# spaceandtimefdn/blitzar

Hardware: NVIDIA H100
Metric: MSM throughput (scalar*point terms/sec), ristretto255, n=2^20 per GPU (higher is better)
Workload: dtype u32 limbs (integer modular arithmetic)

## Files before the change

### blitzar_b200/csrc/msm.cuh

```cuda
#pragma once
#include <algorithm>
#include <vector>

#include "batch_affine.cuh"
#include "curve.cuh"
#include "engine_api.cuh"
#include "lanefield.cuh"

namespace b200 {

struct ColumnDesc {
  const unsigned char* base;
  u64 row_stride;
  u32 bit_offset;
  u32 bit_width;
  u32 n;
  u32 is_signed;
  u32 first_window;
  u32 num_windows;
  u32 table_n;
  u32 gen_base;
};
B200_HD u32 bucket_windows(const ColumnDesc& col) { return col.table_n ? (col.num_windows ? 1u : 0u) : col.num_windows; }

// ... 40 lines not shown
  }
  negative = false;
  if (col.is_signed) {
    u32 top = width - 1;
    bool neg = false;
#pragma unroll
    for (int k = 0; k < 8; ++k)
      if ((top >> 5) == (u32)k)
        neg = (v[k] >> (top & 31u)) & 1u;
    if (neg) {
      u64 c = 1;
#pragma unroll
      for (int k = 0; k < 8; ++k) {
        int lo = 32 * k;
        u32 m = 0;
        if ((int)width >= lo + 32)
          m = 0xffffffffu;
        else if ((int)width > lo)
          m = (1u << (width - lo)) - 1u;
        c += (u64)((~v[k]) & m);
        v[k] = (u32)c & m;
        c = (m == 0xffffffffu) ? (c >> 32) : 0;
      }
      negative = true;
    }
  }
}

constexpr u32 kAllWindows = 0xffffffffu;
template <class Fn>
B200_HD void for_each_digit(const u32 v[8], bool negative, const ColumnDesc& col, u32 c,
                            u32 nbuckets, Fn f, u32 only_window = kAllWindows) {
  const u32 half = nbuckets;
  const u32 mask = (1u << c) - 1u;
  u64 buf = 0;
  u32 nb = 0, w = 0, carry = 0;
  const u32 W = only_window == kAllWindows
                    ? col.num_windows
                    : (only_window < col.num_windows ? only_window + 1 : 0u);
  const auto step = [&] {
    u32 d = ((u32)buf & mask) + carry;
    buf >>= c;
    bool dneg = d > half;
    carry = dneg ? 1u : 0u;
    if (dneg)
      d = (1u << c) - d;
    if (d && (only_window == kAllWindows || w == only_window))
      f((col.first_window + (col.table_n ? 0u : w)) * nbuckets + (d - 1u), negative != dneg, w);
    ++w;
  };
#pragma unroll
  for (int k = 0; k < 8; ++k) {
    buf |= (u64)v[k] << nb;
    nb += 32;
    for (; nb >= c && w < W; nb -= c)
      step();
  }
  while (w < W)
    step();
}

B200_HD u32 column_of(const u64* col_start, u32 ncols, u64 tid) {
  u32 lo = 0, hi = ncols;
  while (hi - lo > 1) {
    const u32 mid = (lo + hi) >> 1;
    if (tid >= col_start[mid])
      lo = mid;
    else
      hi = mid;
  }
  return lo;
}
template <class Fn>
B200_HD void for_each_entry(const ColumnDesc* cols, const u64* col_start, u32 ncols, u32 c,
                            u32 nbuckets, u64 tid, Fn f, u32 only_window = kAllWindows) {
  const u32 j = column_of(col_start, ncols, tid);
  const ColumnDesc col = cols[j];
  if (only_window != kAllWindows && only_window >= col.num_windows)
    return;
  const u64 i = tid - col_start[j];
  u32 v[8];
  bool neg;
  load_scalar_bits(v, neg, col, i);
  const u32 ii = (u32)i + col.gen_base, tn = col.table_n;
  for_each_digit(v, neg, col, c, nbuckets, [&](u32 key, bool negate, u32 w) {
    f(key, make_entry(key, ii + w * tn, negate));
  }, only_window);
}

struct CountBody {
  static constexpr int kBlock = 256;
  const ColumnDesc* cols;
  const u64* col_start;
  u32 ncols, c, nbuckets;
  u32* counts;
  B200_HD void operator()(u64 tid) const {
    u32* cnt = counts;
    for_each_entry(cols, col_start, ncols, c, nbuckets, tid,
                   [cnt](u32 key, u64) { B200_ATOMIC_ADD(&cnt[key], 1u); });
  }
};

struct ScatterBody {
  static constexpr int kBlock = 256;
  const ColumnDesc* cols;
  const u64* col_start;
  u32 ncols, c, nbuckets;
  u32* cursor;
  u64* entries;
  u64 total_terms;
  B200_HD void operator()(u64 tid) const {
    u32 only = kAllWindows;
    if (total_terms) {
      only = (u32)(tid / total_terms);
      tid -= (u64)only * total_terms;
    }
    u32* cur = cursor;
    u64* en = entries;
    for_each_entry(cols, col_start, ncols, c, nbuckets, tid,
                   [cur, en](u32 key, u64 e) { en[B200_ATOMIC_ADD(&cur[key], 1u)] = e; }, only);
  }
};

constexpr u32 kScanChunk = 256, kScanChunkFirst = 64;
struct ScanUpBody {
  static constexpr int kBlock = 128;
  const u32* in;
  u64 n;
  u32* partial;
  u32 chunk;
  B200_HD void operator()(u64 t) const {
    u64 b = t * chunk, e = b + chunk < n ? b + chunk : n;
    u32 s = 0;
    for (u64 i = b; i < e; ++i)
      s += in[i];
    partial[t] = s;
  }
};
struct ScanTopBody {
  static constexpr int kBlock = 32;
  u32* data;
  u64 n;
  B200_HD void operator()(u64) const {
    u32 s = 0;
    for (u64 i = 0; i < n; ++i) {
      u32 v = data[i];
      data[i] = s;
      s += v;
    }
  }
};
struct ScanDownBody {
  static constexpr int kBlock = 128;
  u32* data;
  u64 n;
  const u32* partial_scanned;
  u32 chunk;
  B200_HD void operator()(u64 t) const {
    u64 b = t * chunk, e = b + chunk < n ? b + chunk : n;
    u32 s = partial_scanned[t];
    for (u64 i = b; i < e; ++i) {
      u32 v = data[i];
      data[i] = s;
      s += v;
    }
  }
};

inline void exclusive_scan(u32* data, u64 n, stream_t s, u32 chunk = kScanChunkFirst) {
  if (n <= kScanChunk) {
    launch(ScanTopBody{data, n}, 1, s);
    return;
  }
  u64 m = (n + chunk - 1) / chunk;
  u32* partial = (u32*)dev_alloc(m * sizeof(u32), s);
  launch(ScanUpBody{data, n, partial, chunk}, m, s);
  exclusive_scan(partial, m, s, kScanChunk);
  launch(ScanDownBody{data, n, partial, chunk}, m, s);
  dev_free(partial, s);
}

#if defined(__CUDACC__) && !defined(B200_EMULATE)
#define B200_BINNED_SORT 1
constexpr u32 kMicroBins = 16384, kBinCap = 8192, kBinSpan = 4096, kMaxBinShift = 12;
constexpr u64 kBinnedSortMinEntries = 1ull << 20;

template <int kBlock> __device__ u32 block_exclusive_scan(u32 v, u32* warp_sums, u32* total) {
  const u32 lane = threadIdx.x & 31u, warp = threadIdx.x >> 5;
  u32 x = v;
#pragma unroll
  for (int d = 1; d < 32; d <<= 1) {
    const u32 y = __shfl_up_sync(0xffffffffu, x, d);
    if (lane >= (u32)d)
      x += y;
  }
  if (lane == 31)
    warp_sums[warp] = x;
  __syncthreads();
  if (warp == 0) {
    u32 w = lane < kBlock / 32 ? warp_sums[lane] : 0u;
#pragma unroll
    for (int d = 1; d < 32; d <<= 1) {
      const u32 y = __shfl_up_sync(0xffffffffu, w, d);
      if (lane >= (u32)d)
        w += y;
    }
    if (lane < kBlock / 32)
      warp_sums[lane] = w;
  }
  __syncthreads();
  const u32 pre = (warp ? warp_sums[warp - 1] : 0u) + x - v;
  *total = warp_sums[kBlock / 32 - 1];
  __syncthreads();
  return pre;
}

struct MicroCountBody {
  static constexpr int kBlock = 512;
  const ColumnDesc* cols;
  const u64* col_start;
  u32 ncols, c, nbuckets;
  u64 total_terms;
  u32 tile, shift, nmicro;
  u32* micro_counts;
  __device__ void run(u32 b, unsigned char* smem) const {
    u32* h = (u32*)smem;
    for (u32 m = threadIdx.x; m < nmicro; m += kBlock)
      h[m] = 0;
    __syncthreads();
    const u64 lo = (u64)b * tile, hi = lo + tile < total_terms ? lo + tile : total_terms;
    const u32 sh = shift;
    for (u64 t = lo + threadIdx.x; t < hi; t += kBlock)
      for_each_entry(cols, col_start, ncols, c, nbuckets, t,
                     [h, sh](u32 key, u64) { atomicAdd(&h[key >> sh], 1u); });
    __syncthreads();
    for (u32 m = threadIdx.x; m < nmicro; m += kBlock)
      if (h[m])
        atomicAdd(&micro_counts[m], h[m]);
  }
};

struct PlanBinsBody {
  static constexpr int kBlock = 1024;
  const u32* micro_counts;
  u32 nmicro, span_micro;
  u64 nkeys;
  u32* bin_of;
  u32* bin_start;
  u32* bin_micro;
  u32* bin_cursor;
  u32* nbins_out;
  u32* counts;
  u32* d_m;
  __device__ bool starts_bin(const u32* st, u32 m) const {
    constexpr u32 H = kBinCap / 2;
    return m == 0 || m % span_micro == 0 || micro_counts[m] > H || micro_counts[m - 1] > H ||
           st[m] / H != st[m - 1] / H;
  }
  __device__ void run(u32, unsigned char* smem) const {
    __shared__ u32 ws[32];
    u32* st = (u32*)smem;
    const u32 per = (nmicro + kBlock - 1) / kBlock, m0 = min(threadIdx.x * per, nmicro),
              m1 = min(m0 + per, nmicro);
    u32 sum = 0;
    for (u32 m = m0; m < m1; ++m)
      sum += micro_counts[m];
    u32 total;
    u32 run = block_exclusive_scan<kBlock>(sum, ws, &total);
    for (u32 m = m0; m < m1; ++m) {
      st[m] = run;
      run += micro_counts[m];
    }
    __syncthreads();
    u32 nf = 0;
    for (u32 m = m0; m < m1; ++m)
      nf += starts_bin(st, m) ? 1u : 0u;
    u32 nbins;
    u32 id = block_exclusive_scan<kBlock>(nf, ws, &nbins);
    for (u32 m = m0; m < m1; ++m) {
      if (starts_bin(st, m)) {
        bin_start[id] = st[m];
        bin_micro[id] = m;
        bin_cursor[id] = st[m];
        ++id;
      }
      bin_of[m] = id - 1;
    }
    if (threadIdx.x == 0) {
      bin_start[nbins] = total;
      bin_micro[nbins] = nmicro;
      *nbins_out = nbins;
      counts[nkeys] = total;
      d_m[0] = total;
    }
  }
};

struct CoarseScatterBody {
  static constexpr int kBlock = 1024;
  const ColumnDesc* cols;
  const u64* col_start;
  u32 ncols, c, nbuckets;
  u64 total_terms;
  u32 tile, shift, nmicro;
  const u32* bin_of;
  const u32* nbins_ptr;
  u32* bin_cursor;
  u64* tmp;
  __device__ void run(u32 b, unsigned char* smem) const {
    __shared__ u32 ws[32];
    u32* h = (u32*)smem;
    u32* delta = h + nmicro;
    u64* stage = (u64*)(delta + nmicro + (nmicro & 1u));
    const u32 nbins = *nbins_ptr;
    for (u32 k = threadIdx.x; k < nbins; k += kBlock)
      h[k] = 0;
    __syncthreads();
    const u64 lo = (u64)b * tile, hi = lo + tile < total_terms ? lo + tile : total_terms;
    const u32 sh = shift;
    const u32* map = bin_of;
    for (u64 t = lo + threadIdx.x; t < hi; t += kBlock)
      for_each_entry(cols, col_start, ncols, c, nbuckets, t,
                     [h, sh, map](u32 key, u64) { atomicAdd(&h[__ldg(&map[key >> sh])], 1u); });
    __syncthreads();
    const u32 per = (nbins + kBlock - 1) / kBlock, k0 = min(threadIdx.x * per, nbins),
              k1 = min(k0 + per, nbins);
    u32 sum = 0;
    for (u32 k = k0; k < k1; ++k)
      sum += h[k];
    u32 size;
    u32 run = block_exclusive_scan<kBlock>(sum, ws, &size);
    for (u32 k = k0; k < k1; ++k) {
      const u32 n = h[k];
      if (n)
        delta[k] = atomicAdd(&bin_cursor[k], n) - run;
      h[k] = run;
      run += n;
    }
    __syncthreads();
    for (u64 t = lo + threadIdx.x; t < hi; t += kBlock)
      for_each_entry(cols, col_start, ncols, c, nbuckets, t, [h, sh, map, stage](u32 key, u64 e) {
        stage[atomicAdd(&h[__ldg(&map[key >> sh])], 1u)] = e;
      });
    __syncthreads();
    for (u32 i = threadIdx.x; i < size; i += kBlock) {
      const u64 e = stage[i];
      tmp[delta[__ldg(&map[entry_key(e) >> sh])] + i] = e;
    }
  }
};

struct BinSortBody {
  static constexpr int kBlock = 1024;
  static constexpr size_t kSmem = 2 * kBinCap * sizeof(u64) + kBinSpan * sizeof(u32);
  const u64* tmp;
  const u32* bin_start;
  const u32* bin_micro;
  const u32* nbins_ptr;
  u32 shift;
  u64 nkeys;
  u64* entries;
  u32* counts;
  __device__ void run(u32 b, unsigned char* smem) const {
    __shared__ u32 ws[32];
    if (b >= *nbins_ptr)
      return;
    u64* ent = (u64*)smem;
    u32* h = (u32*)(smem + 2 * kBinCap * sizeof(u64));
    const u32 lo = bin_start[b], size = bin_start[b + 1] - lo;
    const u64 klo = (u64)bin_micro[b] << shift, khi_m = (u64)bin_micro[b + 1] << shift;
    const u32 span = (u32)((khi_m < nkeys ? khi_m : nkeys) - klo);
    const bool local = size <= kBinCap;
    for (u32 k = threadIdx.x; k < span; k += kBlock)
      h[k] = 0;
    if (local) {
#pragma unroll 4
      for (u32 i = threadIdx.x; i < size; i += kBlock)
        ent[i] = tmp[(u64)lo + i];
    }
    __syncthreads();
    for (u32 i = threadIdx.x; i < size; i += kBlock) {
      const u64 e = local ? ent[i] : tmp[(u64)lo + i];
      atomicAdd(&h[entry_key(e) - (u32)klo], 1u);
    }
    __syncthreads();
    const u32 per = (span + kBlock - 1) / kBlock, k0 = min(threadIdx.x * per, span),
              k1 = min(k0 + per, span);
    u32 sum = 0;
    for (u32 k = k0; k < k1; ++k)
      sum += h[k];
    u32 total;
    u32 run = block_exclusive_scan<kBlock>(sum, ws, &total);
    for (u32 k = k0; k < k1; ++k) {
      const u32 n = h[k];
      h[k] = run;
      run += n;
      counts[klo + k] = lo + run;
    }
    __syncthreads();
    if (!local) {
      for (u32 i = threadIdx.x; i < size; i += kBlock) {
        const u64 e = tmp[(u64)lo + i];
        entries[(u64)lo + atomicAdd(&h[entry_key(e) - (u32)klo], 1u)] = e;
      }
      return;
    }
    u64* sorted = ent + kBinCap;
    for (u32 i = threadIdx.x; i < size; i += kBlock) {
      const u64 e = ent[i];
      sorted[atomicAdd(&h[entry_key(e) - (u32)klo], 1u)] = e;
    }
    __syncthreads();
    for (u32 i = threadIdx.x; i < size; i += kBlock)
      entries[(u64)lo + i] = sorted[i];
  }
};

inline u32 binned_sort_shift(u64 nkeys) {
  u32 shift = 0;
  while ((nkeys + (1ull << shift) - 1) >> shift > kMicroBins)
    ++shift;
  return shift;
}

inline void binned_sort(stream_t s, const ColumnDesc* d_cols, const u64* d_col_start, u32 ncols,
                        u32 c, u32 nbuckets, u64 total_terms, u64 max_entries, u32 max_windows,
                        u64 nkeys, u64* entries, u32* counts, u32* d_m) {
  const u32 shift = binned_sort_shift(nkeys);
  const u32 nmicro = (u32)((nkeys + (1ull << shift) - 1) >> shift);
  const u32 span_micro = std::max(1u, kBinSpan >> shift);
  u32* ws = (u32*)dev_alloc((5ull * nmicro + 3) * sizeof(u32), s);
  u32 *micro_counts = ws, *bin_of = ws + nmicro, *bin_cursor = ws + 2ull * nmicro,
      *bin_start = ws + 3ull * nmicro, *bin_micro = ws + 4ull * nmicro + 1,
      *nbins = ws + 5ull * nmicro + 2;
  u64* tmp = (u64*)dev_alloc(std::max<u64>(max_entries, 1) * sizeof(u64), s);
  dev_zero(micro_counts, nmicro * sizeof(u32), s);
  const u64 count_tile = 4096;
  launch_blocks(MicroCountBody{d_cols, d_col_start, ncols, c, nbuckets, total_terms,
                               (u32)count_tile, shift, nmicro, micro_counts},
                (total_terms + count_tile - 1) / count_tile, nmicro * sizeof(u32), s);
  launch_blocks(PlanBinsBody{micro_counts, nmicro, span_micro, nkeys, bin_of, bin_start, bin_micro,
                             bin_cursor, nbins, counts, d_m},
                1, nmicro * sizeof(u32), s);
  const size_t scatter_smem = 220 * 1024;
  const size_t bin_bytes = (2ull * nmicro + 2) * sizeof(u32);
  const u64 stage_entries = (scatter_smem - bin_bytes) / sizeof(u64);
  const u64 scatter_tile = std::max<u64>(1, stage_entries / max_windows);
  launch_blocks(CoarseScatterBody{d_cols, d_col_start, ncols, c, nbuckets, total_terms,
                                  (u32)scatter_tile, shift, nmicro, bin_of, nbins, bin_cursor, tmp},
                (total_terms + scatter_tile - 1) / scatter_tile, scatter_smem, s);
  launch_blocks(BinSortBody{tmp, bin_start, bin_micro, nbins, shift, nkeys, entries, counts}, nmicro,
                BinSortBody::kSmem, s);
  dev_free(tmp, s);
  dev_free(ws, s);
}
#endif

template <class C> struct FillIdentityBody {
  static constexpr int kBlock = 256;
  static constexpr u32 kChunks = sizeof(typename C::Point) / 16;
  static_assert(sizeof(typename C::Point) % 16 == 0, "points are made of 16-byte aligned fields");
  uint4* p;
  B200_HD void operator()(u64 t) const {
    const typename C::Point id = C::identity();
    const u32 k = (u32)(t % kChunks);
    uint4 v = ((const uint4*)&id)[0];
#pragma unroll
    for (u32 j = 1; j < kChunks; ++j)
      if (j == k)
        v = ((const uint4*)&id)[j];
    p[t] = v;
  }
};
template <class C> inline void fill_identity(stream_t s, typename C::Point* p, u64 n) {
  launch(FillIdentityBody<C>{(uint4*)p}, n * FillIdentityBody<C>::kChunks, s);
}

struct BucketOffsets {
  const u32* ends;
  const u32* starts;
  B200_HD u32 begin(u64 k) const { return starts ? starts[k] : (k ? ends[k - 1] : 0u); }
  B200_HD u32 end(u64 k) const { return ends[k]; }
};

template <class C> struct MergeBucketsBody {
  static constexpr int kBlock = 128;
  BucketOffsets offsets;
  const typename C::Point* scratch;
  typename C::Point* buckets;
  B200_HD void operator()(u64 k) const {
    if (offsets.begin(k) == offsets.end(k))
      return;
    typename C::Point b = buckets[k];
    C::add(b, b, scratch[k]);
    buckets[k] = b;
  }
};

template <class C, bool kGather, class X = SeqExec, bool kUniform = false, bool kUnitZ = false>
struct AccumulateBody {
  static constexpr int kBlock = 128;
  static constexpr int kMinBlocks = !kGather ? 1 : (C::F::N > 8 ? 2 : 3);
  typedef typename C::Point Point;
  typedef typename C::Gen Gen;
  const u32* keys;
  const u64* entries;
  const Gen* gens;
  const Point* pieces;
  const u32* m_ptr;
  u32 K;
  u32 final_level;
  Point* buckets;
  u32* out_keys;
  Point* out_pieces;
  u32* out_m_ptr;
  const u32* unit_veto;

  B200_HD void close_run(u64 t, u32 key, const Point& acc, bool writer, bool& first_seg) const {
    if (final_level || !first_seg) {
      if (writer)
        buckets[key] = acc;
    } else if (writer) {
      out_keys[2 * t] = key;
      out_pieces[2 * t] = acc;
    }
    first_seg = false;
  }
  template <bool kUnit> B200_HD Gen load_gen(u32 idx) const {
    if constexpr (kUnit)
      return C::load_unit_gen(gens + idx);
    else
      return gens[idx];
  }
  template <bool kUnit>
  B200_HD void gather_walk(u64 t, u64 b, u64 e, bool writer, u32& cur, Point& acc,
                           bool& first_seg) const {
    u64 ent = entries[b];
    Gen g = load_gen<kUnit>(entry_gen(ent));
    cur = entry_key(ent);
    for (u64 i = b; i < e; ++i) {
      u64 ent_n = ent;
      Gen g_n = g;
      if (i + 1 < e) {
        ent_n = entries[i + 1];
        g_n = load_gen<kUnit>(entry_gen(ent_n));
      }
      const u32 k = entry_key(ent);
      const bool negate = entry_negate(ent);
      if (kUniform) {
        if (i == b || k != cur) {
          if (i != b) {
            close_run(t, cur, acc, writer, first_seg);
            cur = k;
          }
          acc = C::identity();
        }
        C::template add_gen<X>(acc, acc, g, negate, kUnit);
      } else {
        const bool start = i == b || k != cur;
        if (k != cur) {
          close_run(t, cur, acc, writer, first_seg);
          cur = k;
        }
        if (start)
          C::gen_to_point(acc, g, negate);
        else
          C::template add_gen<X>(acc, acc, g, negate, kUnit);
      }
      ent = ent_n;
      g = g_n;
    }
  }
  B200_HD void operator()(u64 tid) const {
    const u64 t = tid / X::kLanes;
    const bool writer = (tid % X::kLanes) == 0;
    const u64 M = *m_ptr;
    const u64 T = (M + K - 1) / K;
    if (tid == 0 && out_m_ptr)
      *out_m_ptr = final_level ? 0u : (u32)(2 * T);
    u64 b = t * K;
    if (b >= M)
      return;
    u64 e = b + K < M ? b + K : M;
    u32 cur;
    Point acc;
    bool first_seg = true;
    if constexpr (kGather) {
      if (kUnitZ && unit_veto && *unit_veto)
        gather_walk<false>(t, b, e, writer, cur, acc, first_seg);
      else
        gather_walk<kUnitZ>(t, b, e, writer, cur, acc, first_seg);
    } else {
      cur = keys[b];
      acc = pieces[b];
      for (u64 i = b + 1; i < e; ++i) {
        const u32 k = keys[i];
        if (k == cur) {
          C::template add<X>(acc, acc, pieces[i]);
        } else {
          close_run(t, cur, acc, writer, first_seg);
          cur = k;
          acc = pieces[i];
        }
      }
    }
    if (final_level) {
      close_run(t, cur, acc, writer, first_seg);
      return;
    }
    if (!writer)
      return;
    if (first_seg) {
      close_run(t, cur, acc, writer, first_seg);
      acc = C::identity();
    }
    out_keys[2 * t + 1] = cur;
    out_pieces[2 * t + 1] = acc;
  }
};

struct WindowUsedBody {
  static constexpr int kBlock = 64;
  BucketOffsets offsets;
  u32 nbuckets;
  u32* window_used;
  B200_HD void operator()(u64 w) const {
    if (offsets.begin(w * nbuckets) != offsets.begin((w + 1) * nbuckets))
      window_used[w] = 1u;
  }
};

template <class C, class Ex = SeqExec> struct ReduceBody {
  static constexpr int kBlock = 64;
  typedef typename C::Point Point;
  const Point* X;
  const Point* Cin;
  u32 m_in, g, log2g;
  Point* Xout;
  Point* Cout;
  const u32* window_used;
  u32 nbuckets;
  B200_HD void operator()(u64 tid) const {
    const u64 t = tid / Ex::kLanes;
    const bool writer = (tid % Ex::kLanes) == 0;
    const u32 m_out = m_in / g;
    const u32 w = (u32)(t / m_out), k = (u32)(t % m_out);
    if (window_used[w] == 0) {
      if (writer) {
        Xout[t] = C::identity();
        Cout[t] = C::identity();
      }
      return;
    }
    const Point* x = X + (u64)w * m_in + (u64)k * g;
    Point run = x[g - 1];
    Point acc = Cin ? C::identity() : run;
    if (Cin) {
      acc = run;
      if (g == 1)
        acc = C::identity();
    }
    for (u32 r = g - 1; r-- > 0;) {
      C::template add<Ex>(run, run, x[r]);
      if (r > 0 || !Cin)
        C::template add<Ex>(acc, acc, run);
    }
    if (Cin) {
      const Point* cin = Cin + (u64)w * m_in + (u64)k * g;
      for (u32 r = 0; r < g; ++r)
        C::template add<Ex>(acc, acc, cin[r]);
    }
    for (u32 i = 0; i < log2g; ++i)
      C::template dbl<Ex>(run, run);
    if (writer) {
      Xout[t] = run;
      Cout[t] = acc;
    }
  }
};

template <class C, class X = SeqExec> struct CombineBody {
  static constexpr int kBlock = 32;
  typedef typename C::Point Point;
  const Point* S;
  const ColumnDesc* cols;
  u32 c;
  Point* out;
  B200_HD void operator()(u64 tid) const {
    const u64 j = tid / X::kLanes;
    const bool writer = (tid % X::kLanes) == 0;
    const ColumnDesc col = cols[j];
    if (col.num_windows == 0 || col.n == 0) {
      if (writer)
        out[j] = C::identity();
      return;
    }
    const u32 nw = bucket_windows(col);
    Point acc = S[col.first_window + nw - 1];
    for (u32 w = nw - 1; w-- > 0;) {
      for (u32 i = 0; i < c; ++i)
        C::template dbl<X>(acc, acc);
      C::template add<X>(acc, acc, S[col.first_window + w]);
    }
    if (writer)
      out[j] = acc;
  }
};

#if defined(__CUDACC__) && !defined(B200_EMULATE)
#define B200_LANE_TAIL 1
struct CombineLaneBody {
  static constexpr int kBlock = 32;
  typedef Ed25519 C;
  const C::Point* S;
  const ColumnDesc* cols;
  u32 c;
  C::Point* out;
  __device__ void operator()(u64 tid) const {
    const u64 j = tid >> 5;
    const ColumnDesc col = cols[j];
    if (col.num_windows == 0 || col.n == 0) {
      if ((tid & 31u) == 0)
        out[j] = C::identity();
      return;
    }
    const lane10::Lane L = lane10::lane_info();
    const u32 nw = bucket_windows(col);
    C::Point acc = S[col.first_window + nw - 1];
    for (u32 w = nw - 1; w-- > 0;) {
      u32 t;
      const u32 v = lane10::dbl_n(L, lane10::slice_point(L, acc), (int)c, t);
      lane10::gather_point(acc, v, t);
      C::add<QuadExecConv>(acc, acc, S[col.first_window + w]);
    }
    if ((tid & 31u) == 0)
      out[j] = acc;
  }
};
struct LanePow {
  static __device__ __forceinline__ void pow22523(F25519::E& r, const F25519::E& a) {
    const lane10::Lane L = lane10::lane_info();
    const u32 g = L.base / 10u;
    lane10::gather(r, lane10::pow22523(L, lane10::slice(L, a)), g < 3 ? g : 0u);
  }
};
struct StoreLaneBody {
  static constexpr int kBlock = 32;
  const Ed25519::Point* pts;
  unsigned char* out;
  u64 count;
  __device__ void operator()(u64 tid) const {
    const u32 lane = (u32)tid & 31u, g = lane / 10u;
    const u64 i = (tid >> 5) * 3 + g;
    const bool live = g < 3 && i < count;
    unsigned char enc[32];
    Ed25519::encode<LanePow>(enc, pts[live ? i : count - 1]);
    if (live && lane == 10u * g) {
      uint4* d = (uint4*)(out + 32 * i);
      const uint4* e = (const uint4*)enc;
      d[0] = e[0];
      d[1] = e[1];
    }
  }
};
#endif

template <class C>
inline void launch_store_commit(stream_t s, const typename C::Point* pts, unsigned char* out,
                                u64 count, bool lane_tail = true);

template <class C, bool kProjective> struct IngestBody {
  static constexpr int kBlock = 128;
  const unsigned char* raw;
  typename C::Gen* gens;
  B200_HD void operator()(u64 i) const {
    typename C::Gen g;
    if (kProjective)
      C::load_proj_abi(g, raw + i * C::kAbiProjBytes);
    else
      C::load_gen_abi(g, raw + i * C::kAbiGenBytes);
    gens[i] = g;
  }
};
constexpr int kMaxTableWindows = 33;
template <class C> struct PrecomputeTableBody {
  static constexpr int kBlock = 64;
  typename C::Gen* table;
  u64 n;
  u32 c, W;
  B200_HD void operator()(u64 i) const {
    typedef typename C::F F;
    typename C::Point p, pts[kMaxTableWindows];
    typename F::E prefix[kMaxTableWindows], acc = F::one(), inv;
    C::gen_to_point(p, table[i], false);
    for (u32 w = 0; w < W; ++w) {
      if (w)
        for (u32 k = 0; k < c; ++k)
          C::dbl(p, p);
      pts[w] = p;
      prefix[w] = acc;
      F::mul(acc, acc, C::denominator(p));
    }
    F::invert(inv, acc);
    for (u32 w = W; w-- > 0;) {
      typename F::E zi;
      F::mul(zi, inv, prefix[w]);
      F::mul(inv, inv, C::denominator(pts[w]));
      typename C::Gen g;
      C::normalized_gen(g, pts[w], zi);
      table[(u64)w * n + i] = g;
    }
  }
};
template <class C> struct IngestCompactBody {
  static constexpr int kBlock = 128;
  const unsigned char* table;
  u32 window_width;
  typename C::Gen* gens;
  B200_HD void operator()(u64 i) const {
    const u64 group = i / window_width, j = i % window_width;
    const u64 entry = (group << window_width) + (1ull << j);
    typename C::Gen g;
    C::load_compact_abi(g, table + entry * C::kAbiCompactBytes);
    gens[i] = g;
  }
};
struct BuiltinGeneratorBody {
  static constexpr int kBlock = 64;
  Ed25519::Gen* gens;
  u64 first;
  B200_HD void operator()(u64 i) const {
    Ed25519::Point g;
    Ed25519::builtin_generator(g, first + i);
    Ed25519::point_to_gen(gens[i], g);
  }
};
struct GenPieces {
  const u64* start;
  const u64* from;
  const u64* to;
  u32 npieces;
};
template <class C> struct IngestPiecesBody {
  static constexpr int kBlock = IngestBody<C, false>::kBlock;
  const unsigned char* raw;
  typename C::Gen* gens;
  GenPieces p;
  B200_HD void operator()(u64 tid) const {
    const u32 k = column_of(p.start, p.npieces, tid);
    IngestBody<C, false>{raw + p.from[k] * C::kAbiGenBytes, gens + p.to[k]}(tid - p.start[k]);
  }
};
struct BuiltinPiecesBody {
  static constexpr int kBlock = BuiltinGeneratorBody::kBlock;
  Ed25519::Gen* gens;
  GenPieces p;
  B200_HD void operator()(u64 tid) const {
    const u32 k = column_of(p.start, p.npieces, tid);
    BuiltinGeneratorBody{gens + p.to[k], p.from[k]}(tid - p.start[k]);
  }
};

struct IngestMap {
  GenPieces p;
  B200_HD void at(u64 i, u64& src, u64& dst) const {
    if (p.npieces == 0) {
      src = dst = i;
      return;
    }
    const u32 k = column_of(p.start, p.npieces, i);
    src = p.from[k] + (i - p.start[k]);
    dst = p.to[k] + (i - p.start[k]);
  }
};
constexpr u32 kNormBlock = 256;
struct NormalizeUpBody {
  static constexpr int kBlock = 128;
  typedef F25519 F;
  const unsigned char* raw;
  IngestMap map;
  u64 n, T;
  F::E* pre;
  F::E* prod;
  u32* invalid;
  B200_HD F::E group(u64 j) const {
    F::E z[kBatchGroup], acc = F::one();
#pragma unroll
    for (u32 k = 0; k < kBatchGroup; ++k) {
      const u64 i = j + k * T;
      z[k] = F::one();
      if (i < n) {
        u64 src, dst;
        map.at(i, src, dst);
        z[k] = Ed25519::load_abi_z(raw + src * Ed25519::kAbiGenBytes);
      }
    }
#pragma unroll
    for (u32 k = 0; k < kBatchGroup; ++k) {
      const u64 i = j + k * T;
      if (i >= n)
        break;
      if (F::is_zero(z[k])) {
        *invalid = 1u;
        z[k] = F::one();
      }
      pre[i] = acc;
      F::mul(acc, acc, z[k]);
    }
    return acc;
  }
  B200_HD void operator()(u64 j) const { prod[j] = group(j); }
};
struct NormalizeDownBody {
  static constexpr int kBlock = 128;
  typedef F25519 F;
  const unsigned char* raw;
  IngestMap map;
  u64 n, T;
  const F::E* pre;
  const F::E* prod;
  const F::E* ps;
  const u32* invalid;
  Ed25519::Gen* gens;
  B200_HD void operator()(u64 j) const {
    const bool scale = *invalid == 0;
    F::E inv = prod[ps ? j / kNormBlock : j];
    if (ps)
      F::mul(inv, inv, ps[j]);
    for (u32 k = kBatchGroup; k-- > 0;) {
      const u64 i = j + k * T;
      if (i >= n)
        continue;
      u64 src, dst;
      map.at(i, src, dst);
      Ed25519::Point p;
      Ed25519::load_point_abi(p, raw + src * Ed25519::kAbiGenBytes);
      if (scale) {
        F::E zi;
        F::mul(zi, inv, pre[i]);
        F::mul(inv, inv, p.Z);
        F::mul(p.X, p.X, zi);
        F::mul(p.Y, p.Y, zi);
        F::mul(p.T, p.T, zi);
        p.Z = F::one();
      }
      Ed25519::Gen g;
      Ed25519::point_to_gen(g, p);
      gens[dst] = g;
    }
  }
};
#ifdef B200_BINNED_SORT
__device__ __forceinline__ F25519::E shfl_up_fe(const F25519::E& a, u32 d) {
  F25519::E r;
#pragma unroll
  for (int k = 0; k < 8; ++k)
    r.l[k] = __shfl_up_sync(0xffffffffu, a.l[k], d);
  return r;
}
__device__ __forceinline__ F25519::E shfl_down_fe(const F25519::E& a, u32 d) {
  F25519::E r;
#pragma unroll
  for (int k = 0; k < 8; ++k)
    r.l[k] = __shfl_down_sync(0xffffffffu, a.l[k], d);
  return r;
}
template <int kBlock>
__device__ void block_prefix_suffix(const F25519::E& x, F25519::E& P, F25519::E& S,
                                    F25519::E& total, F25519::E* ws) {
  typedef F25519 F;
  const u32 lane = threadIdx.x & 31u, warp = threadIdx.x >> 5;
  F::E inc = x, sinc = x;
#pragma unroll
  for (u32 d = 1; d < 32; d <<= 1) {
    const F::E y = shfl_up_fe(inc, d), z = shfl_down_fe(sinc, d);
    if (lane >= d)
      F::mul(inc, inc, y);
    if (lane + d < 32)
      F::mul(sinc, sinc, z);
  }
  F::E pe = shfl_up_fe(inc, 1), se = shfl_down_fe(sinc, 1);
  if (lane == 0)
    pe = F::one();
  if (lane == 31) {
    se = F::one();
    ws[warp] = inc;
  }
  __syncthreads();
  F::E before = F::one(), after = F::one();
  for (u32 w = 0; w < kBlock / 32; ++w) {
    if (w < warp)
      F::mul(before, before, ws[w]);
    else if (w > warp)
      F::mul(after, after, ws[w]);
  }
  F::mul(P, before, pe);
  F::mul(S, se, after);
  F::mul(total, before, ws[warp]);
  F::mul(total, total, after);
  __syncthreads();
}
struct NormalizeUpBlockBody {
  static constexpr int kBlock = kNormBlock;
  typedef F25519 F;
  NormalizeUpBody up;
  F::E* ps;
  F::E* prod;
  __device__ void run(u32 b, unsigned char*) const {
    __shared__ F::E ws[kBlock / 32];
    const u64 j = (u64)b * kBlock + threadIdx.x;
    const F::E g = j < up.T ? up.group(j) : F::one();
    F::E P, S, total;
    block_prefix_suffix<kBlock>(g, P, S, total, ws);
    if (j < up.T)
      F::mul(ps[j], P, S);
    if (threadIdx.x == 0)
      prod[b] = total;
  }
};
struct NormalizeMidBody {
  static constexpr int kBlock = 1024;
  typedef F25519 F;
  F::E* vals;
  F::E* pre;
  u64 m;
  __device__ void run(u32, unsigned char*) const {
    __shared__ F::E ws[kBlock / 32];
    __shared__ F::E inv_total;
    const u64 per = (m + kBlock - 1) / kBlock, lo = min((u64)threadIdx.x * per, m),
              hi = min(lo + per, m);
    F::E c = F::one();
    for (u64 k = lo; k < hi; ++k) {
      pre[k] = c;
      F::mul(c, c, vals[k]);
    }
    F::E P, S, total;
    block_prefix_suffix<kBlock>(c, P, S, total, ws);
    if (threadIdx.x == 0)
      F::invert(inv_total, total);
    __syncthreads();
    F::E inv;
    F::mul(inv, inv_total, P);
    F::mul(inv, inv, S);
    for (u64 k = hi; k-- > lo;) {
      const F::E v = vals[k];
      F::mul(vals[k], inv, pre[k]);
      F::mul(inv, inv, v);
    }
  }
};
#endif
inline void ingest_normalized(stream_t s, const unsigned char* raw, Ed25519::Gen* gens,
                              const IngestMap& map, u64 n, u32* invalid) {
  typedef F25519::E fe;
  if (n == 0)
    return;
  const u64 T = (n + kBatchGroup - 1) / kBatchGroup;
  fe* pre = (fe*)dev_alloc(n * sizeof(fe), s);
  const NormalizeUpBody up{raw, map, n, T, pre, nullptr, invalid};
#ifdef B200_BINNED_SORT
  const u64 blocks = (T + kNormBlock - 1) / kNormBlock;
  fe* ps = (fe*)dev_alloc((T + 2 * blocks) * sizeof(fe), s);
  fe* prod = ps + T;
  launch_blocks(NormalizeUpBlockBody{up, ps, prod}, blocks, 0, s);
  launch_blocks(NormalizeMidBody{prod, prod + blocks, blocks}, 1, 0, s);
  launch(NormalizeDownBody{raw, map, n, T, pre, prod, ps, invalid, gens}, T, s);
  dev_free(ps, s);
#else
  fe* prod = (fe*)dev_alloc(T * sizeof(fe), s);
  NormalizeUpBody u = up;
  u.prod = prod;
  launch(u, T, s);
  batch_invert<F25519>(s, prod, T);
  launch(NormalizeDownBody{raw, map, n, T, pre, prod, nullptr, invalid, gens}, T, s);
  dev_free(prod, s);
#endif
  dev_free(pre, s);
}
template <class C, bool kCommit> struct StoreBody {
  static constexpr int kBlock = 32;
  const typename C::Point* pts;
  unsigned char* out;
  B200_HD void operator()(u64 i) const {
    if (kCommit)
      C::store_commit_abi(out + i * C::kAbiCommitBytes, pts[i]);
    else
      C::store_proj_abi(out + i * C::kAbiProjBytes, pts[i]);
  }
};
template <class C>
inline void launch_store_commit(stream_t s, const typename C::Point* pts, unsigned char* out,
                                u64 count, bool lane_tail) {
#ifdef B200_LANE_TAIL
  if constexpr (C::kCurveId == kRistretto255) {
    if (lane_tail && count && count <= 4096) {
      launch(StoreLaneBody{pts, out, count}, (count + 2) / 3 * 32, s);
      return;
    }
  }
#endif
  launch(StoreBody<C, true>{pts, out}, count, s);
}
template <class C> struct GenToProjBody {
  static constexpr int kBlock = 64;
  const typename C::Gen* gens;
  unsigned char* out;
  B200_HD void operator()(u64 i) const {
    typename C::Point p;
    C::gen_to_point(p, gens[i], false);
    C::store_proj_abi(out + i * C::kAbiProjBytes, p);
  }
};
template <class C> struct SumPartsBody {
  static constexpr int kBlock = 32;
  const typename C::Point* parts;
  u32 nparts, count;
  typename C::Point* out;
  B200_HD void operator()(u64 j) const {
    typename C::Point acc = parts[j];
    for (u32 r = 1; r < nparts; ++r)
      C::add(acc, acc, parts[(u64)r * count + j]);
    out[j] = acc;
  }
};

inline u32 choose_window_bits(u64 max_n, u32 max_width, u32 ncols, size_t point_bytes) {
  const double kMaxBucketBytes = 3.0e9;
  u32 best = 2;
  double best_cost = 1e300;
  for (u32 c = 2; c <= 16; ++c) {
    double W = (double)(max_width / c + 1);
    if (c > 8 && W * (double)(1u << (c - 1)) * (double)ncols * (double)point_bytes > kMaxBucketBytes)
      break;
    double cost = W * ((double)max_n + 2.5 * (double)(1u << (c - 1)));
    if (cost < best_cost) {
      best_cost = cost;
      best = c;
    }
  }
  return best;
}

struct MsmPlan {
  u32 c = 0, nbuckets = 0, ncols = 0, total_windows = 0;
  u64 nkeys = 0, max_n = 0, total_terms = 0, total_entries = 0;
  std::vector<ColumnDesc> cols;
};

inline MsmPlan msm_make_plan(std::vector<ColumnDesc> cols, const MsmOptions& opt,
                             size_t point_bytes) {
  MsmPlan p;
  p.ncols = (u32)cols.size();
  u32 max_width = 1;
  for (auto& col : cols) {
    p.max_n = std::max<u64>(p.max_n, col.n);
    p.total_terms += col.n;
    if (col.n)
      max_width = std::max(max_width, col.bit_width);
  }
  p.c = opt.window_bits ? opt.window_bits
                        : choose_window_bits(p.max_n, max_width, p.ncols, point_bytes);
  p.nbuckets = 1u << (p.c - 1);
  u64 max_entries = 0;
  for (auto& col : cols) {
    col.first_window = p.total_windows;
    col.num_windows = col.n ? col.bit_width / p.c + 1 : 0;
    p.total_windows += bucket_windows(col);
    max_entries += (u64)col.n * col.num_windows;
    if (col.table_n)
      B200_REQUIRE((u64)col.table_n * col.num_windows < (1ull << 31), "generator table too large");
    if (col.n)
      B200_REQUIRE((u64)col.gen_base + col.n + (u64)(col.num_windows - 1) * col.table_n < (1ull << 31),
                   "generator index of a column too large");
  }
  p.nkeys = (u64)p.total_windows * p.nbuckets;
  p.total_entries = max_entries;
  B200_REQUIRE(p.nkeys < (1ull << 32), "too many buckets for one pass");
  p.cols = std::move(cols);
  return p;
}

struct StagedRange {
  const ColumnDesc* d_cols = nullptr;
  const u64* d_col_start = nullptr;
  u64 total_terms = 0, max_entries = 0;
  u32 max_windows = 0;
  StagedRange(stream_t s, const MsmPlan& plan, u64 begin, u64 end) {
    const u32 ncols = plan.ncols;
    std::vector<ColumnDesc> cols(plan.cols);
    std::vector<u64> col_start(ncols + 1, 0);
    for (u32 j = 0; j < ncols; ++j) {
      u64 lo = std::min<u64>(begin, cols[j].n), hi = std::min<u64>(end, cols[j].n);
      cols[j].base += lo * cols[j].row_stride;
      cols[j].n = (u32)(hi - lo);
      col_start[j + 1] = col_start[j] + cols[j].n;
      max_entries += (u64)cols[j].n * cols[j].num_windows;
      max_windows = std::max(max_windows, cols[j].n ? cols[j].num_windows : 0u);
    }
    total_terms = col_start[ncols];
    if (total_terms == 0)
      return;
    B200_REQUIRE(max_entries < (1ull << 32) && end - begin < (1ull << 31),
                 "too many (term, window) entries for one sort pass");
    const size_t desc_bytes = ncols * sizeof(ColumnDesc), start_bytes = (ncols + 1) * sizeof(u64);
    std::vector<unsigned char> stage(desc_bytes + start_bytes);
    std::memcpy(stage.data(), cols.data(), desc_bytes);
    std::memcpy(stage.data() + desc_bytes, col_start.data(), start_bytes);
    d_cols = (const ColumnDesc*)stage_to_device(s, stage.data(), stage.size());
    d_col_start = (const u64*)((const unsigned char*)d_cols + desc_bytes);
  }
};

struct SortedLayout {
  u64* entries;
  u32* counts;
  u32* starts;
  u32* d_m;
  u64 slots_max;
  bool binned;
  BucketOffsets offsets() const { return {counts, starts}; }
};

inline SortedLayout sort_entries(stream_t s, const MsmPlan& plan, const StagedRange& r, u32 L,
                                 const MsmOptions& opt, u32* window_used) {
  const u32 ncols = plan.ncols, c = plan.c, nbuckets = plan.nbuckets;
  const u64 nkeys = plan.nkeys, max_entries = r.max_entries, total_terms = r.total_terms;
  SortedLayout out{};
  out.slots_max = L ? ((max_entries + nkeys * ((1ull << L) - 1) + (1ull << L) - 1) >> L) << L : max_entries;
  out.counts = (u32*)dev_alloc((nkeys + 1) * sizeof(u32), s);
  out.d_m = (u32*)dev_alloc(16 * sizeof(u32), s);
  out.entries = (u64*)dev_alloc(out.slots_max * sizeof(u64), s);
#ifdef B200_BINNED_SORT
  out.binned = L == 0 && opt.sort_path != 0 && binned_sort_shift(nkeys) <= kMaxBinShift &&
               (opt.sort_path == 2 || max_entries >= kBinnedSortMinEntries);
  if (out.binned)
    binned_sort(s, r.d_cols, r.d_col_start, ncols, c, nbuckets, total_terms, max_entries,
                r.max_windows, nkeys, out.entries, out.counts, out.d_m);
#endif
  if (!out.binned) {
    dev_zero(out.counts, (nkeys + 1) * sizeof(u32), s);
    launch(CountBody{r.d_cols, r.d_col_start, ncols, c, nbuckets, out.counts}, total_terms, s);
    if (L)
      launch(PadCountsBody{out.counts, (1u << L) - 1u}, nkeys, s);
    exclusive_scan(out.counts, nkeys + 1, s);
    copy_d2d(out.d_m, out.counts + nkeys, sizeof(u32), s);
    if (L) {
      out.starts = (u32*)dev_alloc((nkeys + 1) * sizeof(u32), s);
      copy_d2d(out.starts, out.counts, (nkeys + 1) * sizeof(u32), s);
    }
    const bool window_major = opt.scatter_window_major && r.max_windows > 1;
    launch(ScatterBody{r.d_cols, r.d_col_start, ncols, c, nbuckets, out.counts, out.entries,
                       window_major ? total_terms : 0},
           window_major ? total_terms * r.max_windows : total_terms, s);
  }
  if (L)
    launch(FillPadsBody{out.starts, out.counts, out.entries}, nkeys, s);
  launch(WindowUsedBody{out.offsets(), nbuckets, window_used}, plan.total_windows, s);
  return out;
}

inline unsigned sort_selftest(stream_t s, std::vector<ColumnDesc> cols, u32 c) {
  MsmOptions opt;
  opt.window_bits = c;
  const MsmPlan plan = msm_make_plan(std::move(cols), opt, 160);
  const StagedRange r(s, plan, 0, plan.max_n);
  if (r.total_terms == 0)
    return ~0u;
  const u64 nkeys = plan.nkeys, M = r.max_entries;
  DevBuf<u32> window_used(plan.total_windows, s);
  opt.sort_path = 0;
  const SortedLayout a = sort_entries(s, plan, r, 0, opt, window_used.p);
  opt.sort_path = 2;
  const SortedLayout b = sort_entries(s, plan, r, 0, opt, window_used.p);
  std::vector<u32> ca(nkeys + 1), cb(nkeys + 1), m(1);
  std::vector<u64> ea(M), eb(M);
  copy_d2h(ca.data(), a.counts, (nkeys + 1) * sizeof(u32), s);
  copy_d2h(cb.data(), b.counts, (nkeys + 1) * sizeof(u32), s);
  copy_d2h(m.data(), b.d_m, sizeof(u32), s);
  copy_d2h(ea.data(), a.entries, M * sizeof(u64), s);
  copy_d2h(eb.data(), b.entries, M * sizeof(u64), s);
  stream_sync(s);
  for (void* p : {(void*)a.entries, (void*)a.counts, (void*)a.d_m, (void*)b.entries, (void*)b.counts,
                  (void*)b.d_m, (void*)r.d_cols})
    dev_free(p, s);
  if (!b.binned)
    return ~0u;
  unsigned bad = m[0] == ca[nkeys] ? 0u : 1u;
  for (u64 k = 0; k < nkeys; ++k) {
    const u32 lo = k ? ca[k - 1] : 0u, hi = ca[k];
    if (cb[k] != hi || hi < lo || hi > M) {
      ++bad;
      continue;
    }
    std::sort(ea.begin() + lo, ea.begin() + hi);
    std::sort(eb.begin() + lo, eb.begin() + hi);
    if (!std::equal(ea.begin() + lo, ea.begin() + hi, eb.begin() + lo))
      ++bad;
  }
  return bad;
}

struct RangeHook {
  virtual void before_range(u64 begin, u64 end) = 0;
  virtual void before_accumulate() {}
  virtual ~RangeHook() {}
};

template <class C>
stream_t chunk_walk(stream_t s, stream_t tail, WalkInput<C> walk, u32* d_m, bool unit,
                    const u32* unit_veto, typename C::Point* target, const MsmOptions& opt,
                    std::vector<void*>& to_free) {
  typedef typename C::Point Point;
  u32 K = opt.chunk1 ? std::max(opt.chunk1, 4u) : (walk.m_max >= (1ull << 23) ? 64u : 32u);
  const u32 chunkn = std::max(opt.chunkn, 4u);
  const u32* lvl_keys = nullptr;
  const Point* lvl_pieces = nullptr;
  stream_t cs = s;
  for (int level = 0;; ++level) {
    const bool final_level = walk.m_max <= K;
    u64 T = (walk.m_max + K - 1) / K;
    u32* out_keys = final_level ? nullptr : (u32*)dev_alloc(2 * T * sizeof(u32), cs);
    Point* out_pieces = final_level ? nullptr : (Point*)dev_alloc(2 * T * sizeof(Point), cs);
    to_free.insert(to_free.end(), {out_keys, out_pieces});
    u32* out_m = d_m + 1 + (level % 8);
    const auto launch_level = [&](auto body, u64 threads, stream_t st) {
      body = {lvl_keys, walk.entries, walk.gens, lvl_pieces, walk.m_ptr, K, final_level, target,
              out_keys, out_pieces, out_m, unit_veto};
      launch(body, threads, st);
    };
    if (level == 0) {
      const bool uniform =
          opt.uniform_add == 2 ? C::kCurveId == kRistretto255 : opt.uniform_add != 0;
      constexpr bool kEd = C::kCurveId == kRistretto255;
      const bool unit_path = kEd && unit;
      if (uniform && unit_path)
        launch_level(AccumulateBody<C, true, SeqExec, true, kEd>{}, T, s);
      else if (uniform)
        launch_level(AccumulateBody<C, true, SeqExec, true>{}, T, s);
      else if (unit_path)
        launch_level(AccumulateBody<C, true, SeqExec, false, kEd>{}, T, s);
      else
        launch_level(AccumulateBody<C, true>{}, T, s);
// ... 190 lines not shown
```

### blitzar_b200/csrc/runtime.cuh

```cuda
#pragma once
#include <cstdio>
#include <cstdlib>
#include <cstring>
#include <atomic>
#include <cctype>
#include <string>
#include <utility>
#include <vector>

#include "field.cuh"

#ifndef B200_EMULATE
#include <cuda_runtime.h>
#include <nvtx3/nvToolsExt.h>
#endif

namespace b200 {

[[noreturn]] inline void die(const char* what, const char* file, int line) {
  std::fprintf(stderr, "blitzar_b200: fatal: %s (%s:%d)\n", what, file, line);
  std::abort();
}
#define B200_REQUIRE(cond, msg)                                                                    \
  do {                                                                                             \
    if (!(cond))                                                                                   \
      ::b200::die(msg, __FILE__, __LINE__);                                                        \
  } while (0)

inline int log_level() {
  static const int level = [] {
    const char* env = std::getenv("BLITZAR_LOG_LEVEL");
    if (!env)
      return 0;
    std::string s(env);
    for (auto& ch : s)
      ch = (char)std::tolower((unsigned char)ch);
    if (s == "warn")
      return 1;
    if (s == "info")
      return 2;
    if (s == "debug" || s == "trace")
      return 3;
    return 0;
  }();
  return level;
}
#define B200_LOG(level, ...)                                                                       \
  do {                                                                                             \
    if (::b200::log_level() >= (level)) {                                                          \
      std::fprintf(stderr, "[blitzar_b200] " __VA_ARGS__);                                         \
      std::fputc('\n', stderr);                                                                    \
    }                                                                                              \
  } while (0)

struct StageRange {
#ifndef B200_EMULATE
  explicit StageRange(const char* name) { nvtxRangePushA(name); }
  ~StageRange() { nvtxRangePop(); }
#else
  explicit StageRange(const char*) {}
#endif
  StageRange(const StageRange&) = delete;
  StageRange& operator=(const StageRange&) = delete;
};

#ifndef B200_EMULATE
#define B200_CUDA(call)                                                                            \
  do {                                                                                             \
    cudaError_t e_ = (call);                                                                       \
    if (e_ != cudaSuccess)                                                                         \
      ::b200::die(cudaGetErrorString(e_), __FILE__, __LINE__);                                     \
  } while (0)

typedef cudaStream_t stream_t;

template <class Body, class = void> struct MinBlocks {
  static constexpr int value = 1;
};
template <class Body> struct MinBlocks<Body, decltype((void)Body::kMinBlocks)> {
  static constexpr int value = Body::kMinBlocks;
};
template <class Body>
__global__ void __launch_bounds__(Body::kBlock, MinBlocks<Body>::value) k_run(Body body, u64 n) {
  u64 tid = (u64)blockIdx.x * blockDim.x + threadIdx.x;
  if (tid < n)
    body(tid);
}

struct LaunchCounter {
  static std::atomic<unsigned long long>& value() {
    static std::atomic<unsigned long long> v{0};
    return v;
  }
};

template <class Body> inline void launch(const Body& body, u64 n, stream_t s) {
  if (n == 0)
    return;
  u64 blocks = (n + Body::kBlock - 1) / Body::kBlock;
  B200_REQUIRE(blocks < (1ull << 31), "grid too large");
  k_run<Body><<<(unsigned)blocks, Body::kBlock, 0, s>>>(body, n);
  B200_CUDA(cudaGetLastError());
  ++LaunchCounter::value();
}
template <class Body> __global__ void __launch_bounds__(Body::kBlock) k_block(Body body) {
  extern __shared__ __align__(16) unsigned char smem[];
  body.run(blockIdx.x, smem);
}
template <class Body>
inline void launch_blocks(const Body& body, u64 blocks, size_t smem_bytes, stream_t s) {
  if (blocks == 0)
    return;
  B200_REQUIRE(blocks < (1ull << 31), "grid too large");
  static thread_local size_t raised = 48 * 1024;
  if (smem_bytes > raised) {
    B200_CUDA(cudaFuncSetAttribute(k_block<Body>, cudaFuncAttributeMaxDynamicSharedMemorySize,
                                   (int)smem_bytes));
    raised = smem_bytes;
  }
  k_block<Body><<<(unsigned)blocks, Body::kBlock, smem_bytes, s>>>(body);
  B200_CUDA(cudaGetLastError());
  ++LaunchCounter::value();
}
inline void* dev_alloc(size_t bytes, stream_t s) {
  void* p = nullptr;
  B200_CUDA(cudaMallocAsync(&p, bytes ? bytes : 16, s));
  return p;
}
inline void dev_free(void* p, stream_t s) {
  if (p)
    B200_CUDA(cudaFreeAsync(p, s));
}
inline void dev_zero(void* p, size_t bytes, stream_t s) { B200_CUDA(cudaMemsetAsync(p, 0, bytes, s)); }
inline void copy_h2d(void* d, const void* h, size_t bytes, stream_t s) {
  if (bytes)
    B200_CUDA(cudaMemcpyAsync(d, h, bytes, cudaMemcpyHostToDevice, s));
}
inline void copy_d2h(void* h, const void* d, size_t bytes, stream_t s) {
  if (bytes)
    B200_CUDA(cudaMemcpyAsync(h, d, bytes, cudaMemcpyDeviceToHost, s));
}
inline void copy_d2d(void* d, const void* s_, size_t bytes, stream_t s) {
  if (bytes)
    B200_CUDA(cudaMemcpyAsync(d, s_, bytes, cudaMemcpyDeviceToDevice, s));
}
inline void stream_sync(stream_t s) { B200_CUDA(cudaStreamSynchronize(s)); }
inline void stream_follow(stream_t later, stream_t earlier) {
  static thread_local cudaEvent_t ring[64];
  static thread_local unsigned next = 0;
  cudaEvent_t& e = ring[next++ % 64];
  if (!e)
    B200_CUDA(cudaEventCreateWithFlags(&e, cudaEventDisableTiming));
  B200_CUDA(cudaEventRecord(e, earlier));
  B200_CUDA(cudaStreamWaitEvent(later, e, 0));
}

inline stream_t aux_stream() {
  static thread_local cudaStream_t s = nullptr;
  if (!s)
    B200_CUDA(cudaStreamCreateWithFlags(&s, cudaStreamNonBlocking));
  return s;
}

struct StagingRing {
  static constexpr size_t kSlotBytes = 65536, kSlots = 128;
  unsigned char* base = nullptr;
  cudaEvent_t done[kSlots];
  size_t next = 0;
  static StagingRing& get() {
    static thread_local StagingRing r;
    return r;
  }
  void* stage(stream_t s, const void* host, size_t bytes) {
    void* d = dev_alloc(bytes, s);
    if (bytes > kSlotBytes) {
      copy_h2d(d, host, bytes, s);
      stream_sync(s);
      return d;
    }
    if (!base) {
      B200_CUDA(cudaHostAlloc((void**)&base, kSlotBytes * kSlots, cudaHostAllocDefault));
      for (auto& e : done) {
        B200_CUDA(cudaEventCreateWithFlags(&e, cudaEventDisableTiming));
      }
    }
    size_t slot = next++ % kSlots;
    B200_CUDA(cudaEventSynchronize(done[slot]));
    std::memcpy(base + slot * kSlotBytes, host, bytes);
    B200_CUDA(cudaMemcpyAsync(d, base + slot * kSlotBytes, bytes, cudaMemcpyHostToDevice, s));
    B200_CUDA(cudaEventRecord(done[slot], s));
    return d;
  }
};
inline void* stage_to_device(stream_t s, const void* host, size_t bytes) {
  return StagingRing::get().stage(s, host, bytes);
}

struct KernelTimer {
  bool enabled = false;
  std::vector<std::pair<cudaEvent_t, cudaEvent_t>> spans;
  static KernelTimer& get() {
    static thread_local KernelTimer t;
    return t;
  }
  void begin(stream_t s) {
    if (!enabled)
      return;
    cudaEvent_t a, b;
    B200_CUDA(cudaEventCreate(&a));
    B200_CUDA(cudaEventCreate(&b));
    B200_CUDA(cudaEventRecord(a, s));
    spans.emplace_back(a, b);
  }
  void end(stream_t s) {
    if (!enabled)
      return;
    B200_CUDA(cudaEventRecord(spans.back().second, s));
  }
  void read(float* total_ms, unsigned* count) {
    float tot = 0;
    for (auto& sp : spans) {
      float ms = 0;
      B200_CUDA(cudaEventSynchronize(sp.second));
      B200_CUDA(cudaEventElapsedTime(&ms, sp.first, sp.second));
      tot += ms;
      B200_CUDA(cudaEventDestroy(sp.first));
      B200_CUDA(cudaEventDestroy(sp.second));
    }
    *total_ms = tot;
    *count = (unsigned)spans.size();
    spans.clear();
  }
};
template <class T> B200_HD T atomic_add(T* p, T v) {
#ifdef __CUDA_ARCH__
  return atomicAdd(p, v);
#else
  T old = *p;
  *p = old + v;
  return old;
#endif
}
#define B200_ATOMIC_ADD(ptr, v) ::b200::atomic_add((ptr), (v))
#else
typedef int stream_t;
struct LaunchCounter {
  static unsigned long long& value() {
    static unsigned long long v = 0;
    return v;
  }
};
template <class Body> inline void launch(const Body& body, u64 n, stream_t) {
  for (u64 t = 0; t < n; ++t)
    body(t);
  ++LaunchCounter::value();
}
inline void* dev_alloc(size_t bytes, stream_t) { return std::malloc(bytes ? bytes : 16); }
inline void dev_free(void* p, stream_t) { std::free(p); }
inline void dev_zero(void* p, size_t bytes, stream_t) { std::memset(p, 0, bytes); }
inline void copy_h2d(void* d, const void* h, size_t bytes, stream_t) { std::memcpy(d, h, bytes); }
inline void copy_d2h(void* h, const void* d, size_t bytes, stream_t) { std::memcpy(h, d, bytes); }
inline void copy_d2d(void* d, const void* s_, size_t bytes, stream_t) { std::memcpy(d, s_, bytes); }
inline void stream_sync(stream_t) {}
inline void stream_follow(stream_t, stream_t) {}
inline stream_t aux_stream() { return 0; }
inline void* stage_to_device(stream_t s, const void* host, size_t bytes) {
  void* d = dev_alloc(bytes, s);
  std::memcpy(d, host, bytes);
  return d;
}
struct KernelTimer {
  static KernelTimer& get() {
    static KernelTimer t;
    return t;
  }
  void begin(stream_t) {}
  void end(stream_t) {}
};
template <class T> inline T emul_atomic_add(T* p, T v) {
  T old = *p;
  *p = old + v;
  return old;
}
#define B200_ATOMIC_ADD(ptr, v) ::b200::emul_atomic_add((ptr), (v))
#endif

}
```

Before: 351.5 million.

## Shrink bin-sort block and smem, size scatter tiles by live bins, warp-parallel inversion

BinSortBody moves to 512-thread blocks with a min-blocks launch bound and keeps each thread's entries in registers, not a second shared-memory buffer. That halves its shared-memory footprint so two blocks can share an SM. CoarseScatterBody now sizes its tile from the runtime bin count instead of the worst-case micro-bin count, giving more staging space per block, though blocks past the end just exit. NormalizeMid's single-thread field inversion becomes a warp-cooperative lane10 exponentiation.

```diff
diff --git a/blitzar_b200/csrc/msm.cuh b/blitzar_b200/csrc/msm.cuh
--- a/blitzar_b200/csrc/msm.cuh
+++ b/blitzar_b200/csrc/msm.cuh
@@ -366,21 +366,25 @@
   const u64* col_start;
   u32 ncols, c, nbuckets;
   u64 total_terms;
-  u32 tile, shift, nmicro;
+  u32 smem_words, max_windows, shift;
   const u32* bin_of;
   const u32* nbins_ptr;
   u32* bin_cursor;
   u64* tmp;
+  B200_HD u32 tile(u32 nbins) const { return (smem_words - nbins) / max_windows; }
   __device__ void run(u32 b, unsigned char* smem) const {
     __shared__ u32 ws[32];
+    const u32 nbins = *nbins_ptr;
+    const u64 lo = (u64)b * tile(nbins);
+    if (lo >= total_terms)
+      return;
+    const u64 hi = lo + tile(nbins) < total_terms ? lo + tile(nbins) : total_terms;
     u32* h = (u32*)smem;
-    u32* delta = h + nmicro;
-    u64* stage = (u64*)(delta + nmicro + (nmicro & 1u));
-    const u32 nbins = *nbins_ptr;
+    u32* delta = h + nbins;
+    u64* stage = (u64*)(delta + nbins);
     for (u32 k = threadIdx.x; k < nbins; k += kBlock)
       h[k] = 0;
     __syncthreads();
-    const u64 lo = (u64)b * tile, hi = lo + tile < total_terms ? lo + tile : total_terms;
     const u32 sh = shift;
     const u32* map = bin_of;
     for (u64 t = lo + threadIdx.x; t < hi; t += kBlock)
@@ -415,8 +419,9 @@
 };
 
 struct BinSortBody {
-  static constexpr int kBlock = 1024;
-  static constexpr size_t kSmem = 2 * kBinCap * sizeof(u64) + kBinSpan * sizeof(u32);
+  static constexpr int kBlock = 512, kMinBlocks = 2;
+  static constexpr u32 kPer = kBinCap / kBlock;
+  static constexpr size_t kSmem = kBinCap * sizeof(u64) + kBinSpan * sizeof(u32);
   const u64* tmp;
   const u32* bin_start;
   const u32* bin_micro;
@@ -429,23 +434,31 @@
     __shared__ u32 ws[32];
     if (b >= *nbins_ptr)
       return;
-    u64* ent = (u64*)smem;
-    u32* h = (u32*)(smem + 2 * kBinCap * sizeof(u64));
+    u64* sorted = (u64*)smem;
+    u32* h = (u32*)(smem + kBinCap * sizeof(u64));
     const u32 lo = bin_start[b], size = bin_start[b + 1] - lo;
     const u64 klo = (u64)bin_micro[b] << shift, khi_m = (u64)bin_micro[b + 1] << shift;
     const u32 span = (u32)((khi_m < nkeys ? khi_m : nkeys) - klo);
     const bool local = size <= kBinCap;
+    u64 e[kPer];
+    const auto load = [&](u32 base) {
+#pragma unroll
+      for (u32 j = 0; j < kPer; ++j)
+        if (base + threadIdx.x + j * kBlock < size)
+          e[j] = tmp[(u64)lo + base + threadIdx.x + j * kBlock];
+    };
+    if (local)
+      load(0);
     for (u32 k = threadIdx.x; k < span; k += kBlock)
       h[k] = 0;
-    if (local) {
-#pragma unroll 4
-      for (u32 i = threadIdx.x; i < size; i += kBlock)
-        ent[i] = tmp[(u64)lo + i];
-    }
     __syncthreads();
-    for (u32 i = threadIdx.x; i < size; i += kBlock) {
-      const u64 e = local ? ent[i] : tmp[(u64)lo + i];
-      atomicAdd(&h[entry_key(e) - (u32)klo], 1u);
+    for (u32 base = 0; base < size; base += kBinCap) {
+      if (!local)
+        load(base);
+#pragma unroll
+      for (u32 j = 0; j < kPer; ++j)
+        if (base + threadIdx.x + j * kBlock < size)
+          atomicAdd(&h[entry_key(e[j]) - (u32)klo], 1u);
     }
     __syncthreads();
     const u32 per = (span + kBlock - 1) / kBlock, k0 = min(threadIdx.x * per, span),
@@ -463,17 +476,19 @@
     }
     __syncthreads();
     if (!local) {
-      for (u32 i = threadIdx.x; i < size; i += kBlock) {
-        const u64 e = tmp[(u64)lo + i];
-        entries[(u64)lo + atomicAdd(&h[entry_key(e) - (u32)klo], 1u)] = e;
+      for (u32 base = 0; base < size; base += kBinCap) {
+        load(base);
+#pragma unroll
+        for (u32 j = 0; j < kPer; ++j)
+          if (base + threadIdx.x + j * kBlock < size)
+            entries[(u64)lo + atomicAdd(&h[entry_key(e[j]) - (u32)klo], 1u)] = e[j];
       }
       return;
     }
-    u64* sorted = ent + kBinCap;
-    for (u32 i = threadIdx.x; i < size; i += kBlock) {
-      const u64 e = ent[i];
-      sorted[atomicAdd(&h[entry_key(e) - (u32)klo], 1u)] = e;
-    }
+#pragma unroll
+    for (u32 j = 0; j < kPer; ++j)
+      if (threadIdx.x + j * kBlock < size)
+        sorted[atomicAdd(&h[entry_key(e[j]) - (u32)klo], 1u)] = e[j];
     __syncthreads();
     for (u32 i = threadIdx.x; i < size; i += kBlock)
       entries[(u64)lo + i] = sorted[i];
@@ -507,12 +522,12 @@
                              bin_cursor, nbins, counts, d_m},
                 1, nmicro * sizeof(u32), s);
   const size_t scatter_smem = 220 * 1024;
-  const size_t bin_bytes = (2ull * nmicro + 2) * sizeof(u32);
-  const u64 stage_entries = (scatter_smem - bin_bytes) / sizeof(u64);
-  const u64 scatter_tile = std::max<u64>(1, stage_entries / max_windows);
-  launch_blocks(CoarseScatterBody{d_cols, d_col_start, ncols, c, nbuckets, total_terms,
-                                  (u32)scatter_tile, shift, nmicro, bin_of, nbins, bin_cursor, tmp},
-                (total_terms + scatter_tile - 1) / scatter_tile, scatter_smem, s);
+  const CoarseScatterBody scatter{d_cols, d_col_start, ncols, c, nbuckets, total_terms,
+                                  (u32)(scatter_smem / sizeof(u64)), max_windows, shift, bin_of,
+                                  nbins, bin_cursor, tmp};
+  B200_REQUIRE(scatter.tile(nmicro) > 0, "too many windows per term for the binned sort");
+  launch_blocks(scatter, (total_terms + scatter.tile(nmicro) - 1) / scatter.tile(nmicro),
+                scatter_smem, s);
   launch_blocks(BinSortBody{tmp, bin_start, bin_micro, nbins, shift, nkeys, entries, counts}, nmicro,
                 BinSortBody::kSmem, s);
   dev_free(tmp, s);
@@ -1100,8 +1115,15 @@
     }
     F::E P, S, total;
     block_prefix_suffix<kBlock>(c, P, S, total, ws);
-    if (threadIdx.x == 0)
-      F::invert(inv_total, total);
+    if (threadIdx.x < 32) {
+      const lane10::Lane L = lane10::lane_info();
+      const u32 a = lane10::slice(L, total);
+      const u32 t = lane10::sqr_n(L, lane10::pow22523(L, a), 3);
+      F::E r;
+      lane10::gather(r, lane10::mul(L, t, lane10::mul(L, lane10::mul(L, a, a), a)), 0);
+      if (threadIdx.x == 0)
+        inv_total = r;
+    }
     __syncthreads();
     F::E inv;
     F::mul(inv, inv_total, P);
diff --git a/blitzar_b200/csrc/runtime.cuh b/blitzar_b200/csrc/runtime.cuh
--- a/blitzar_b200/csrc/runtime.cuh
+++ b/blitzar_b200/csrc/runtime.cuh
@@ -103,7 +103,8 @@
   B200_CUDA(cudaGetLastError());
   ++LaunchCounter::value();
 }
-template <class Body> __global__ void __launch_bounds__(Body::kBlock) k_block(Body body) {
+template <class Body>
+__global__ void __launch_bounds__(Body::kBlock, MinBlocks<Body>::value) k_block(Body body) {
   extern __shared__ __align__(16) unsigned char smem[];
   body.run(blockIdx.x, smem);
 }
```

After: 369.8 million (median of 6 runs). +5.2%, better.
